# naba89/EDM-TTS

Measured on NVIDIA B200. Metric: s2a_decoded_codec_frames_per_s, higher is better.
Workload: dtype bf16

## Files before the change

edm_tts_b200/csrc/abi.cu:

```cuda
#include <atomic>
#include <cmath>
#include <cstdarg>
#include <cstdio>
#include <cstdlib>
#include <cstring>
#include <string>
#include <algorithm>
#include <utility>
#include <vector>

#include "../../include/edm_s2a.h"
#include "attention.cuh"
#include "elementwise.cuh"
#include "conv_stream.cuh"
#include "dac_conv.cuh"
#include "gemm.cuh"
#include "kmeans.cuh"
#include "rvq_tc.cuh"

using namespace edm;

namespace {

thread_local char g_err[512] = "";
// ... 135 lines not shown
  cfg.stream = st;
  cudaLaunchAttribute attr[1];
  attr[0].id = cudaLaunchAttributeProgrammaticStreamSerialization;
  attr[0].val.programmaticStreamSerializationAllowed = 1;
  cfg.attrs = attr;
  cfg.numAttrs = pdl_enabled() ? 1 : 0;
  cudaLaunchKernelEx(&cfg, kernel, std::forward<Args>(args)...);
}

typedef CUresult (*PFN_tmapEncodeTiled)(CUtensorMap*, CUtensorMapDataType, cuuint32_t, void*, const cuuint64_t*, const cuuint64_t*,
                                        const cuuint32_t*, const cuuint32_t*, CUtensorMapInterleave, CUtensorMapSwizzle,
                                        CUtensorMapL2promotion, CUtensorMapFloatOOBfill);
PFN_tmapEncodeTiled get_encode() {
  static PFN_tmapEncodeTiled fn = nullptr;
  if (fn == nullptr) {
    void* p = nullptr;
    cudaDriverEntryPointQueryResult q;
    if (cudaGetDriverEntryPoint("cuTensorMapEncodeTiled", &p, cudaEnableDefault, &q) == cudaSuccess && q == cudaDriverEntryPointSuccess)
      fn = reinterpret_cast<PFN_tmapEncodeTiled>(p);
  }
  return fn;
}

int make_tmap_2d(CUtensorMap* m, const void* ptr, uint64_t rows, uint64_t cols, uint64_t ld, uint32_t box_rows) {
  PFN_tmapEncodeTiled enc = get_encode();
  if (enc == nullptr) return fail(EDM_ERR_CUDA, "cuTensorMapEncodeTiled entry point not available");
  if ((reinterpret_cast<uintptr_t>(ptr) & 15) != 0 || (ld * 2) % 16 != 0) return fail(EDM_ERR_INVALID, "TMA operand must be 16-byte aligned (ptr %p, ld %llu)", ptr, (unsigned long long)ld);
  cuuint64_t dims[2] = {cols, rows};
  cuuint64_t strides[1] = {ld * 2};
  cuuint32_t box[2] = {64, box_rows};
  cuuint32_t estr[2] = {1, 1};
  CUresult r = enc(m, CU_TENSOR_MAP_DATA_TYPE_BFLOAT16, 2, const_cast<void*>(ptr), dims, strides, box, estr, CU_TENSOR_MAP_INTERLEAVE_NONE,
                   CU_TENSOR_MAP_SWIZZLE_128B, CU_TENSOR_MAP_L2_PROMOTION_L2_256B, CU_TENSOR_MAP_FLOAT_OOB_FILL_NONE);
  if (r != CUDA_SUCCESS) return fail(EDM_ERR_CUDA, "cuTensorMapEncodeTiled(2d rows=%llu cols=%llu ld=%llu) failed: %d", (unsigned long long)rows, (unsigned long long)cols, (unsigned long long)ld, (int)r);
  return 0;
}
int make_tmap_f32_2d(CUtensorMap* m, const void* ptr, uint64_t rows, uint64_t cols, uint64_t ld, uint32_t box_rows,
                     CUtensorMapSwizzle swizzle = CU_TENSOR_MAP_SWIZZLE_128B) {
  PFN_tmapEncodeTiled enc = get_encode();
  if (enc == nullptr) return fail(EDM_ERR_CUDA, "cuTensorMapEncodeTiled entry point not available");
  if ((reinterpret_cast<uintptr_t>(ptr) & 15) != 0 || (ld * 4) % 16 != 0) return fail(EDM_ERR_INVALID, "TMA operand must be 16-byte aligned (ptr %p, ld %llu)", ptr, (unsigned long long)ld);
  cuuint64_t dims[2] = {cols, rows};
  cuuint64_t strides[1] = {ld * 4};
  cuuint32_t box[2] = {32, box_rows};
  cuuint32_t estr[2] = {1, 1};
  CUresult r = enc(m, CU_TENSOR_MAP_DATA_TYPE_FLOAT32, 2, const_cast<void*>(ptr), dims, strides, box, estr, CU_TENSOR_MAP_INTERLEAVE_NONE,
                   swizzle, CU_TENSOR_MAP_L2_PROMOTION_L2_256B, CU_TENSOR_MAP_FLOAT_OOB_FILL_NONE);
  if (r != CUDA_SUCCESS) return fail(EDM_ERR_CUDA, "cuTensorMapEncodeTiled(f32 rows=%llu cols=%llu ld=%llu) failed: %d", (unsigned long long)rows, (unsigned long long)cols, (unsigned long long)ld, (int)r);
  return 0;
}

int next_direction() {
  static const bool enabled = env_switch("EDM_FLIP", true);
  thread_local int dir = 0;
  if (!enabled) return 0;
  dir ^= 1;
  return dir;
}

struct WMap {
  CUtensorMap big, small;
};
int make_wmap(WMap* m, const void* ptr, uint64_t rows, uint64_t cols, uint64_t ld) {
  if (rows % kGemmBN == 0) {
    if (int rc = make_tmap_2d(&m->big, ptr, rows, cols, ld, kGemmBN / 2)) return rc;
  } else {
    memset(&m->big, 0, sizeof(m->big));
  }
  return make_tmap_2d(&m->small, ptr, rows, cols, ld, kSmBN);
}
bool gemm_small_m() { static const bool v = env_switch("EDM_GEMM_SMALL", true); return v; }
bool gemm_resid_tma() { static const bool v = env_switch("EDM_RESID_TMA", true); return v; }
int resid_tma_max_k() { static const int v = env_int("EDM_RESID_TMA_MAXK", 2048); return v; }
bool gemm_out_tma() { static const bool v = env_switch("EDM_OUT_TMA", true); return v; }

template <int EPI>
int launch_gemm_t(const CUtensorMap& ma, const WMap& wm, const GemmParams& p_in, cudaStream_t st) {
  const CUtensorMap& mb = wm.big;
  GemmParams p = p_in;
  p.reverse = next_direction();
  static DeviceOnce attr_once;
  if (attr_once.needed()) {
    EDM_CUDA(cudaFuncSetAttribute(gemm_bf16_tn_pair_kernel<EPI>, cudaFuncAttributeMaxDynamicSharedMemorySize, kPairSmemBytes));
    EDM_CUDA(cudaFuncSetAttribute(gemm_bf16_tn_small_kernel<EPI>, cudaFuncAttributeMaxDynamicSharedMemorySize, kSmSmemBytes));
    if (EPI == EPI_RESID_F32)
      EDM_CUDA(cudaFuncSetAttribute(gemm_bf16_tn_pair_kernel<EPI_RESID_TMA>, cudaFuncAttributeMaxDynamicSharedMemorySize, kPairSmemBytes));
    if (EPI == EPI_SWISH_BF16)
      EDM_CUDA(cudaFuncSetAttribute(gemm_bf16_tn_pair_kernel<EPI_SWISH_TMA>, cudaFuncAttributeMaxDynamicSharedMemorySize, kPairSmemBytes));
    if (EPI == EPI_QKV_ROPE)
      EDM_CUDA(cudaFuncSetAttribute(gemm_bf16_tn_pair_kernel<EPI_ROPE_TMA>, cudaFuncAttributeMaxDynamicSharedMemorySize, kPairSmemBytes));
    if (EPI == EPI_F32)
      EDM_CUDA(cudaFuncSetAttribute(gemm_bf16_tn_pair_kernel<EPI_F32_TMA>, cudaFuncAttributeMaxDynamicSharedMemorySize, kPairSmemBytes));
    attr_once.done();
  }
  ProfScope prof(PK_GEMM, 2.0 * p.M * p.N * p.K, st);
  const int sms = num_sms();
  {
    const int pair_tiles = ((p.M + 2 * kGemmBM - 1) / (2 * kGemmBM)) * ((p.N + kGemmBN - 1) / kGemmBN);
    if (p.N % kGemmBN != 0 || (gemm_small_m() && pair_tiles * 4 <= sms)) {
      p.reverse = 0;
      const int tiles = ((p.M + kGemmBM - 1) / kGemmBM) * (p.N / kSmBN);
      launch_pdl(gemm_bf16_tn_small_kernel<EPI>, dim3(tiles < sms ? tiles : sms), dim3(kSmThreads), kSmSmemBytes, st, ma, wm.small, p);
      EDM_LAUNCH_CHECK("gemm_bf16_tn_small");
      return 0;
    }
  }
  const int tiles = ((p.M + 2 * kGemmBM - 1) / (2 * kGemmBM)) * (p.N / kGemmBN);
  const int pairs = tiles < sms / 2 ? tiles : sms / 2;
  if (EPI == EPI_RESID_F32 && gemm_resid_tma() && p.K <= resid_tma_max_k() && (reinterpret_cast<uintptr_t>(p.out) & 15) == 0 && (p.ldo * 4) % 16 == 0) {
    CUtensorMap mc;
    if (int rc = make_tmap_f32_2d(&mc, p.out, p.M, p.N, p.ldo, 32, CU_TENSOR_MAP_SWIZZLE_128B)) return rc;
    launch_pdl(gemm_bf16_tn_pair_kernel<EPI_RESID_TMA>, dim3(2 * pairs), dim3(kGemmThreads), kPairSmemBytes, st, ma, mb, mc, p);
  } else if (EPI == EPI_F32 && gemm_out_tma() && (reinterpret_cast<uintptr_t>(p.out) & 15) == 0 && (p.ldo * 4) % 16 == 0) {
    CUtensorMap mc;
    if (int rc = make_tmap_f32_2d(&mc, p.out, p.M, p.N, p.ldo, 32, CU_TENSOR_MAP_SWIZZLE_128B)) return rc;
    launch_pdl(gemm_bf16_tn_pair_kernel<EPI_F32_TMA>, dim3(2 * pairs), dim3(kGemmThreads), kPairSmemBytes, st, ma, mb, mc, p);
  } else if ((EPI == EPI_SWISH_BF16 || EPI == EPI_QKV_ROPE) && gemm_out_tma() && (reinterpret_cast<uintptr_t>(p.out) & 15) == 0 && (p.ldo * 2) % 16 == 0) {
    CUtensorMap mc;
    if (int rc = make_tmap_2d(&mc, p.out, p.M, p.N, p.ldo, 32)) return rc;
    if (EPI == EPI_SWISH_BF16)
      launch_pdl(gemm_bf16_tn_pair_kernel<EPI_SWISH_TMA>, dim3(2 * pairs), dim3(kGemmThreads), kPairSmemBytes, st, ma, mb, mc, p);
    else
      launch_pdl(gemm_bf16_tn_pair_kernel<EPI_ROPE_TMA>, dim3(2 * pairs), dim3(kGemmThreads), kPairSmemBytes, st, ma, mb, mc, p);
  } else {
    launch_pdl(gemm_bf16_tn_pair_kernel<EPI>, dim3(2 * pairs), dim3(kGemmThreads), kPairSmemBytes, st, ma, mb, ma, p);
  }
  EDM_LAUNCH_CHECK("gemm_bf16_tn_pair");
  return 0;
}
int launch_gemm(int epi, const CUtensorMap& ma, const WMap& mb, const GemmParams& p, cudaStream_t st) {
  if (p.M <= 0 || p.N <= 0 || p.N % kSmBN != 0 || p.N > kGemmMaxN || p.K % kGemmBK != 0 || p.K <= 0) return fail(EDM_ERR_INVALID, "gemm shape M=%d N=%d K=%d unsupported (N %% 64, N <= 8192, K %% 64)", p.M, p.N, p.K);
  switch (epi) {
    case EPI_BF16: return launch_gemm_t<EPI_BF16>(ma, mb, p, st);
    case EPI_SWISH_BF16: return launch_gemm_t<EPI_SWISH_BF16>(ma, mb, p, st);
    case EPI_QKV_ROPE: return launch_gemm_t<EPI_QKV_ROPE>(ma, mb, p, st);
    case EPI_RESID_F32: return launch_gemm_t<EPI_RESID_F32>(ma, mb, p, st);
    case EPI_F32: return launch_gemm_t<EPI_F32>(ma, mb, p, st);
    case EPI_GLU_BF16: return launch_gemm_t<EPI_GLU_BF16>(ma, mb, p, st);
    case EPI_ARGMAX: return launch_gemm_t<EPI_ARGMAX>(ma, mb, p, st);
  }
  return fail(EDM_ERR_INVALID, "unknown epilogue %d", epi);
}

#ifdef EDM_ATTN_TRACE
unsigned long long* g_attn_trace = nullptr;
#endif
int launch_attention(const CUtensorMap& mqkv, const SeqLayout& lay, const int* pairs, int n_pairs, double flops, int H, void* out, uint32_t lbo,
                     uint32_t sbo, uint32_t kstep, cudaStream_t st, float scale = 0.125f) {
// ... 179 lines not shown
  for (auto& e : g_prof) {
    g_event_pool.push_back(e.a);
    g_event_pool.push_back(e.b);
  }
  g_prof.clear();
  g_prof_on = on != 0;
}
extern "C" int edm_prof_collect(double* ms, double* work, int* count) {
  for (int k = 0; k < PK_COUNT; ++k) {
    ms[k] = 0.0;
    work[k] = 0.0;
    count[k] = 0;
  }
  for (auto& e : g_prof) {
    EDM_CUDA(cudaEventSynchronize(e.b));
    float t = 0.f;
    EDM_CUDA(cudaEventElapsedTime(&t, e.a, e.b));
    ms[e.kind] += t;
    work[e.kind] += e.work;
    count[e.kind] += 1;
  }
  return 0;
}

#ifdef EDM_KTRACE
extern "C" int edm_ktrace_dump(unsigned long long* host, int max_slots) {
  unsigned n = 0;
  cudaDeviceSynchronize();
  cudaMemcpyFromSymbol(&n, g_ktrace_n, sizeof(n));
  const int m = static_cast<int>(n) < max_slots ? static_cast<int>(n) : max_slots;
  if (host != nullptr && m > 0) cudaMemcpyFromSymbol(host, g_ktrace, sizeof(unsigned long long) * 8 * (m < 4096 ? m : 4096));
  const unsigned zero = 0;
  cudaMemcpyToSymbol(g_ktrace_n, &zero, sizeof(zero));
  return static_cast<int>(n);
}
#endif

extern "C" int edm_gemm_bf16(const void* a, long long lda, const void* b, long long ldb, int M, int N, int K, int epilogue,
                             const float* bias, void* out, long long ldo, float scale, const float* rope_cos,
                             const float* rope_sin, int seq_len, int rope_cols, void* stream) {
  if (int rc = check_arch()) return rc;
  CUtensorMap ma;
  WMap mb;
  if (int rc = make_tmap_2d(&ma, a, M, K, lda, kGemmBM)) return rc;
  if (int rc = make_wmap(&mb, b, N, K, ldb)) return rc;
  GemmParams p;
// ... 1722 lines not shown
```

edm_tts_b200/csrc/gemm.cuh:

```cuda
#pragma once
#include "ptx.cuh"
#include "seq_layout.cuh"

namespace edm {

enum EpiKind : int {
  EPI_BF16 = 0,
  EPI_SWISH_BF16 = 1,
  EPI_QKV_ROPE = 2,
  EPI_RESID_F32 = 3,
  EPI_F32 = 4,
  EPI_GLU_BF16 = 5,
  EPI_ARGMAX = 10,
  EPI_F32_TMA = 9,
  EPI_ROPE_TMA = 8,
  EPI_SWISH_TMA = 7,
  EPI_RESID_TMA = 6,
};

struct GemmParams {
  int M, N, K;
  int a_k_offset;
  int b_row_offset;
  const float* bias;
// ... 70 lines not shown
  for (int i = 0; i < 32; ++i)
    if (b[i] > best) {
      best = b[i];
      idx = 32 + i;
    }
  float2* o = reinterpret_cast<float2*>(p.out) + static_cast<long long>(row) * p.ldo + (col >> 6);
  *o = make_float2(best, __int_as_float(col + idx));
}

__device__ __forceinline__ void gemm_store_glu(const GemmParams& p, int row, int col_out, const float (&a)[32], const float (&g)[32]) {
  uint32_t w[16];
#pragma unroll
  for (int i = 0; i < 16; ++i) {
    const uint32_t a2 = pack_bf16x2(a[2 * i], a[2 * i + 1]);
    const uint32_t g2 = pack_bf16x2(g[2 * i], g[2 * i + 1]);
    const uint32_t s2 = pack_bf16x2(sigmoid_tanh(bf16lo(g2)), sigmoid_tanh(bf16hi(g2)));
    w[i] = bf16x2_mul(a2, s2);
  }
  uint4* o = reinterpret_cast<uint4*>(static_cast<__nv_bfloat16*>(p.out) + static_cast<long long>(row) * p.ldo + col_out);
#pragma unroll
  for (int i = 0; i < 4; ++i) o[i] = make_uint4(w[4 * i], w[4 * i + 1], w[4 * i + 2], w[4 * i + 3]);
}

__device__ __forceinline__ void gemm_epilogue_rope64(const GemmParams& p, int row, int col, const uint32_t (&lo)[32],
                                                     const uint32_t (&hi)[32], uint32_t tab_row = 0, int swz = 0, uint32_t stg_row = 0) {
  uint4* o = reinterpret_cast<uint4*>(static_cast<__nv_bfloat16*>(p.out) + static_cast<long long>(row) * p.ldo + col);
  auto put = [&](int c, uint4 v) {
    if (stg_row != 0)
      sts128(stg_row + ((c ^ swz) << 4), make_float4(__uint_as_float(v.x), __uint_as_float(v.y), __uint_as_float(v.z), __uint_as_float(v.w)));
    else
      o[c] = v;
  };
  uint32_t l2[16], h2[16];
#pragma unroll
  for (int i = 0; i < 16; ++i) {
    l2[i] = pack_bf16x2(__uint_as_float(lo[2 * i]), __uint_as_float(lo[2 * i + 1]));
    h2[i] = pack_bf16x2(__uint_as_float(hi[2 * i]), __uint_as_float(hi[2 * i + 1]));
  }
  if (col < p.rope_cols) {
    const int pos = rope_pos(p, row);
    const float4* c4 = reinterpret_cast<const float4*>(p.rope_cos + static_cast<long long>(pos) * 32);
    const float4* s4 = reinterpret_cast<const float4*>(p.rope_sin + static_cast<long long>(pos) * 32);
#pragma unroll
    for (int g = 0; g < 4; ++g) {
      float4 cs[2], sn[2];
      if (tab_row != 0) {
        cs[0] = lds128(tab_row + 16 * ((2 * g) ^ swz));
        cs[1] = lds128(tab_row + 16 * ((2 * g + 1) ^ swz));
        sn[0] = lds128(tab_row + 16 * (8 + ((2 * g) ^ swz)));
        sn[1] = lds128(tab_row + 16 * (8 + ((2 * g + 1) ^ swz)));
      } else {
        cs[0] = __ldg(c4 + 2 * g);
        cs[1] = __ldg(c4 + 2 * g + 1);
        sn[0] = __ldg(s4 + 2 * g);
        sn[1] = __ldg(s4 + 2 * g + 1);
      }
      uint32_t ol[4], oh[4];
#pragma unroll
      for (int q = 0; q < 4; ++q) {
        const int i = 4 * g + q;
        const float4 c = cs[q >> 1], s = sn[q >> 1];
        const float c0 = (q & 1) ? c.z : c.x, c1 = (q & 1) ? c.w : c.y;
        const float s0 = (q & 1) ? s.z : s.x, s1 = (q & 1) ? s.w : s.y;
        const float x1a = bf16lo(l2[i]), x1b = bf16hi(l2[i]), x2a = bf16lo(h2[i]), x2b = bf16hi(h2[i]);
        ol[q] = pack_bf16x2(__fadd_rn(__fmul_rn(x1a, c0), __fmul_rn(-x2a, s0)), __fadd_rn(__fmul_rn(x1b, c1), __fmul_rn(-x2b, s1)));
        oh[q] = pack_bf16x2(__fadd_rn(__fmul_rn(x2a, c0), __fmul_rn(x1a, s0)), __fadd_rn(__fmul_rn(x2b, c1), __fmul_rn(x1b, s1)));
      }
      put(g, make_uint4(ol[0], ol[1], ol[2], ol[3]));
      put(4 + g, make_uint4(oh[0], oh[1], oh[2], oh[3]));
    }
  } else {
#pragma unroll
    for (int g = 0; g < 4; ++g) {
      put(g, make_uint4(l2[4 * g], l2[4 * g + 1], l2[4 * g + 2], l2[4 * g + 3]));
      put(4 + g, make_uint4(h2[4 * g], h2[4 * g + 1], h2[4 * g + 2], h2[4 * g + 3]));
    }
  }
}

constexpr int kSmBN = 64;
constexpr int kSmStages = 8;
constexpr int kSmThreads = 64 + 32 * 4;
constexpr uint32_t kSmBBytes = kSmBN * kGemmBK * 2;
constexpr uint32_t kSmStageBytes = kGemmABytes + kSmBBytes;
constexpr uint32_t kSmSmemBytes = kSmStages * kSmStageBytes + 1024 + 256;

template <int EPI>
__global__ void __launch_bounds__(kSmThreads, 1)
gemm_bf16_tn_small_kernel(const __grid_constant__ CUtensorMap tma_a, const __grid_constant__ CUtensorMap tma_b, const GemmParams p) {
  extern __shared__ uint8_t smem_raw[];
  uint8_t* smem = reinterpret_cast<uint8_t*>((reinterpret_cast<uintptr_t>(smem_raw) + 1023) & ~static_cast<uintptr_t>(1023));
  uint64_t* full_bar = reinterpret_cast<uint64_t*>(smem + kSmStages * kSmStageBytes);
  uint64_t* empty_bar = full_bar + kSmStages;
  uint64_t* tmem_full_bar = empty_bar + kSmStages;
  uint64_t* tmem_empty_bar = tmem_full_bar + 2;
  uint32_t* tmem_base_slot = reinterpret_cast<uint32_t*>(tmem_empty_bar + 2);

  const int warp = threadIdx.x >> 5;
  const int lane = threadIdx.x & 31;
  const int num_m = (p.M + kGemmBM - 1) / kGemmBM;
// ... 99 lines not shown
      }
      if constexpr (EPI != EPI_QKV_ROPE) {
        const float4* bg = reinterpret_cast<const float4*>(p.bias != nullptr ? p.bias + col0 : nullptr);
#pragma unroll
        for (int i = 0; i < 16; ++i) bias_v[i] = bg != nullptr ? __ldg(bg + i) : make_float4(0.f, 0.f, 0.f, 0.f);
      }
      mbar_wait(&tmem_full_bar[acc], acc_phase);
      tc_fence_after();
      uint32_t r0[32], r1[32];
      tmem_ld_32x32(taddr, r0);
      tmem_ld_32x32(taddr + 32, r1);
      tmem_ld_wait_dep(r0);
      tmem_ld_wait_dep(r1);
      tc_fence_before();
      __syncwarp();
#ifdef EDM_KTRACE
      if (warp == 2 && lane == 0) KTRACE_PUT(5, ktrace_now());
#endif
      if (lane == 0) mbar_arrive(&tmem_empty_bar[acc]);
      acc ^= 1;
      if (acc == 0) acc_phase ^= 1;
      if (row >= p.M) continue;
      if constexpr (EPI == EPI_QKV_ROPE) {
        gemm_epilogue_rope64(p, row, col0, r0, r1);
      } else {
        auto bias4 = [&](int i) { return bias_v[i]; };
        float v[32];
#pragma unroll
        for (int i = 0; i < 8; ++i) {
          const float4 b = bias4(i);
          v[4 * i + 0] = __uint_as_float(r0[4 * i + 0]) + b.x;
          v[4 * i + 1] = __uint_as_float(r0[4 * i + 1]) + b.y;
          v[4 * i + 2] = __uint_as_float(r0[4 * i + 2]) + b.z;
          v[4 * i + 3] = __uint_as_float(r0[4 * i + 3]) + b.w;
        }
        if constexpr (EPI == EPI_GLU_BF16 || EPI == EPI_ARGMAX) {
          float g[32];
#pragma unroll
          for (int i = 0; i < 8; ++i) {
            const float4 b = bias4(8 + i);
            g[4 * i + 0] = __uint_as_float(r1[4 * i + 0]) + b.x;
            g[4 * i + 1] = __uint_as_float(r1[4 * i + 1]) + b.y;
            g[4 * i + 2] = __uint_as_float(r1[4 * i + 2]) + b.z;
            g[4 * i + 3] = __uint_as_float(r1[4 * i + 3]) + b.w;
          }
          if constexpr (EPI == EPI_GLU_BF16)
            gemm_store_glu(p, row, col0 >> 1, v, g);
// ... 6 lines not shown
#pragma unroll
          for (int i = 0; i < 8; ++i) {
            const float4 b = bias4(8 + i);
            v[4 * i + 0] = __uint_as_float(r1[4 * i + 0]) + b.x;
            v[4 * i + 1] = __uint_as_float(r1[4 * i + 1]) + b.y;
            v[4 * i + 2] = __uint_as_float(r1[4 * i + 2]) + b.z;
            v[4 * i + 3] = __uint_as_float(r1[4 * i + 3]) + b.w;
          }
          gemm_store_32<EPI>(q, row, col0 + 32, v);
        }
      }
    }
  }

  tc_fence_before();
  __syncthreads();
#ifdef EDM_KTRACE
  if (threadIdx.x == 64) KTRACE_END(100 + EPI);
#endif
  if (warp == 1) tmem_dealloc<128>(tmem_base);
}

constexpr uint32_t kPairStageBytes = 2 * kGemmABytes;
constexpr uint32_t kPairStagingBytes = 32 * 32 * 4;
constexpr uint32_t kPairRopeTabBytes = 128 * 16 * 16;
constexpr uint32_t kPairBarOffset = 7 * kPairStageBytes;
constexpr uint32_t kPairSmemBytes = kPairBarOffset + 256 + 1024;
__host__ __device__ constexpr int pair_stages(bool tma_out, bool rope) { return rope ? (tma_out ? 4 : 6) : (tma_out ? 5 : 7); }
constexpr int kPairMaxStages = 7;

template <int EPI>
__global__ void __cluster_dims__(2, 1, 1) __launch_bounds__(kGemmThreads, 1)
gemm_bf16_tn_pair_kernel(const __grid_constant__ CUtensorMap tma_a, const __grid_constant__ CUtensorMap tma_b,
                         const __grid_constant__ CUtensorMap tma_c, const GemmParams p) {
  constexpr bool kTmaOut = EPI == EPI_RESID_TMA || EPI == EPI_SWISH_TMA || EPI == EPI_ROPE_TMA || EPI == EPI_F32_TMA;
  constexpr bool kRope = EPI == EPI_QKV_ROPE || EPI == EPI_ROPE_TMA;
  constexpr int kSt = pair_stages(kTmaOut, kRope);
  constexpr uint32_t kStagingOffset = kSt * kPairStageBytes;
  constexpr uint32_t kRopeTabOffset = kStagingOffset + (kTmaOut ? kGemmEpiWarps * kPairStagingBytes : 0);
  static_assert(kRopeTabOffset + (kRope ? kPairRopeTabBytes : 0) <= kPairBarOffset, "smem budget");
  extern __shared__ uint8_t smem_raw[];
  uint8_t* smem = reinterpret_cast<uint8_t*>((reinterpret_cast<uintptr_t>(smem_raw) + 1023) & ~static_cast<uintptr_t>(1023));
  float* s_rope = reinterpret_cast<float*>(smem + kRopeTabOffset);
  uint64_t* full_bar = reinterpret_cast<uint64_t*>(smem + kPairBarOffset);
  uint64_t* empty_bar = full_bar + kPairMaxStages;
  uint64_t* tmem_full_bar = empty_bar + kPairMaxStages;
  uint64_t* tmem_empty_bar = tmem_full_bar + 2;
  uint32_t* tmem_base_slot = reinterpret_cast<uint32_t*>(tmem_empty_bar + 2);

  const int warp = threadIdx.x >> 5;
  const int lane = threadIdx.x & 31;
  const uint32_t rank = cluster_ctarank();
  const int pair = blockIdx.x >> 1, num_pairs = gridDim.x >> 1;

  const int num_m = (p.M + 2 * kGemmBM - 1) / (2 * kGemmBM);
  const int num_n = p.N / kGemmBN;
  const int num_tiles = num_m * num_n;
  const int num_kb = p.K / kGemmBK;

  if (warp == 0 && lane == 0) {
    tma_prefetch_desc(&tma_a);
    tma_prefetch_desc(&tma_b);
    for (int s = 0; s < kSt; ++s) {
      mbar_init(&full_bar[s], 1);
      mbar_init(&empty_bar[s], 1);
    }
    for (int b = 0; b < 2; ++b) {
      mbar_init(&tmem_full_bar[b], 1);
      mbar_init(&tmem_empty_bar[b], 2 * kGemmEpiWarps);
    }
    fence_mbar_init();
  }
  if (warp == 1) tmem_alloc_pair<512>(tmem_base_slot);
  tc_fence_before();
  cluster_sync_all();
  tc_fence_after();
  const uint32_t tmem_base = *tmem_base_slot;
  pdl_sync();

  if (warp == 0) {
    if (lane == 0) {
      int stage = 0;
      uint32_t phase = 0;
      for (int t = pair; t < num_tiles; t += num_pairs) {
        const int tt = p.reverse ? num_tiles - 1 - t : t;
        const int m_blk = tt / num_n, n_blk = tt % num_n;
        for (int kb = 0; kb < num_kb; ++kb) {
          mbar_wait(&empty_bar[stage], phase ^ 1);
          uint8_t* sa = smem + stage * kPairStageBytes;
          uint8_t* sb = sa + kGemmABytes;
          if (rank == 0) mbar_arrive_expect_tx(&full_bar[stage], 2 * kPairStageBytes);
          tma_load_2d_pair(&tma_a, &full_bar[stage], sa, p.a_k_offset + kb * kGemmBK, m_blk * 2 * kGemmBM + rank * kGemmBM);
          tma_load_2d_pair(&tma_b, &full_bar[stage], sb, kb * kGemmBK, p.b_row_offset + n_blk * kGemmBN + rank * (kGemmBN / 2));
          if (++stage == kSt) {
            stage = 0;
            phase ^= 1;
          }
        }
      }
    }
  } else if (warp == 1) {
    if (rank == 0) {
      constexpr uint32_t idesc = umma_idesc_bf16(2 * kGemmBM, kGemmBN, 0, 0);
      int stage = 0;
      uint32_t phase = 0;
      int acc = 0;
      uint32_t acc_phase = 0;
      for (int t = pair; t < num_tiles; t += num_pairs) {
        mbar_wait(&tmem_empty_bar[acc], acc_phase ^ 1);
        tc_fence_after();
        const uint32_t d_tmem = tmem_base + acc * kGemmBN;
        for (int kb = 0; kb < num_kb; ++kb) {
          mbar_wait(&full_bar[stage], phase);
          tc_fence_after();
          const uint32_t sa = smem_u32(smem + stage * kPairStageBytes);
          const uint64_t adesc = umma_desc_sw128(sa, 16, 1024);
          const uint64_t bdesc = umma_desc_sw128(sa + kGemmABytes, 16, 1024);
#pragma unroll
          for (int k = 0; k < kGemmBK / 16; ++k) umma_ss_pair_warp(d_tmem, adesc + 2 * k, bdesc + 2 * k, idesc, (kb | k) != 0 ? 1u : 0u);
          umma_commit_pair_warp(&empty_bar[stage]);
          if (++stage == kSt) {
            stage = 0;
            phase ^= 1;
          }
        }
        umma_commit_pair_warp(&tmem_full_bar[acc]);
        acc ^= 1;
        if (acc == 0) acc_phase ^= 1;
      }
    }
  } else {
    const int quad = warp & 3;
    const int sub = (warp - 2) >> 2;
    int acc = 0;
    uint32_t acc_phase = 0;
    for (int t = pair; t < num_tiles; t += num_pairs) {
      const int tt = p.reverse ? num_tiles - 1 - t : t;
      const int m_blk = tt / num_n, n_blk = tt % num_n;
      const int row = m_blk * 2 * kGemmBM + static_cast<int>(rank) * kGemmBM + quad * 32 + lane;
      const int col0 = n_blk * kGemmBN + sub * 64;
      const uint32_t taddr = tmem_base + (static_cast<uint32_t>(quad * 32) << 16) + acc * kGemmBN + sub * 64;
      const float4* bias_g = reinterpret_cast<const float4*>(p.bias != nullptr ? p.bias + col0 : nullptr);
      auto bias4 = [&](int k) { return bias_g != nullptr ? __ldg(bias_g + k) : make_float4(0.f, 0.f, 0.f, 0.f); };
      bool rope_tile = false;
      if constexpr (kRope) {
        rope_tile = n_blk * kGemmBN < p.rope_cols;
        if (rope_tile) {
          float4* tab = reinterpret_cast<float4*>(s_rope);
          const int et = threadIdx.x - 64;
          asm volatile("bar.sync 1, 512;" ::: "memory");
#pragma unroll
          for (int i = et; i < 128 * 16; i += 32 * kGemmEpiWarps) {
            const int r = i >> 4, c = i & 15;
            const int grow = m_blk * 2 * kGemmBM + static_cast<int>(rank) * kGemmBM + r;
            const int pos = rope_pos(p, grow < p.M ? grow : 0);
            const float* src = (c < 8 ? p.rope_cos : p.rope_sin) + static_cast<long long>(pos) * 32 + (c & 7) * 4;
            tab[r * 16 + (c ^ (r & 7))] = __ldg(reinterpret_cast<const float4*>(src));
          }
          asm volatile("bar.sync 1, 512;" ::: "memory");
        }
      }
      mbar_wait(&tmem_full_bar[acc], acc_phase);
      tc_fence_after();
      uint32_t r0[32], r1[32];
      tmem_ld_32x32(taddr, r0);
      tmem_ld_32x32(taddr + 32, r1);
      tmem_ld_wait_dep(r0);
      tmem_ld_wait_dep(r1);
      tc_fence_before();
      __syncwarp();
      if (lane == 0) mbar_arrive_cluster(&tmem_empty_bar[acc], 0);
      acc ^= 1;
      if (acc == 0) acc_phase ^= 1;
      if constexpr (EPI == EPI_ROPE_TMA) {
        uint8_t* stg = smem + kStagingOffset + (warp - 2) * kPairStagingBytes;
        const int tr = quad * 32 + lane;
        if (lane == 0) bulk_wait_group_read0();
        __syncwarp();
        gemm_epilogue_rope64(p, row, col0, r0, r1, rope_tile ? smem_u32(s_rope) + tr * 256 : 0u, tr & 7, smem_u32(stg) + lane * 128);
        fence_proxy_async_smem();
        __syncwarp();
        if (lane == 0) {
          tma_store_2d(&tma_c, stg, col0, m_blk * 2 * kGemmBM + static_cast<int>(rank) * kGemmBM + quad * 32);
          bulk_commit_group();
        }
        continue;
      }
      if constexpr (EPI == EPI_SWISH_TMA) {
        uint8_t* stg = smem + kStagingOffset + (warp - 2) * kPairStagingBytes;
        const uint32_t stg_row = smem_u32(stg) + lane * 128;
        const int sw = lane & 7;
        const int row0 = m_blk * 2 * kGemmBM + static_cast<int>(rank) * kGemmBM + quad * 32;
        uint32_t w[32];
#pragma unroll
        for (int h = 0; h < 2; ++h) {
          const uint32_t* r = h == 0 ? r0 : r1;
#pragma unroll
          for (int i = 0; i < 8; ++i) {
            const float4 b = bias4(8 * h + i);
            const uint32_t h01 = pack_bf16x2(__uint_as_float(r[4 * i + 0]) + b.x, __uint_as_float(r[4 * i + 1]) + b.y);
            const uint32_t h23 = pack_bf16x2(__uint_as_float(r[4 * i + 2]) + b.z, __uint_as_float(r[4 * i + 3]) + b.w);
            w[16 * h + 2 * i] = bf16x2_mul(h01, pack_bf16x2(sigmoid_tanh(bf16lo(h01)), sigmoid_tanh(bf16hi(h01))));
            w[16 * h + 2 * i + 1] = bf16x2_mul(h23, pack_bf16x2(sigmoid_tanh(bf16lo(h23)), sigmoid_tanh(bf16hi(h23))));
          }
        }
        if (lane == 0) bulk_wait_group_read0();
        __syncwarp();
#pragma unroll
        for (int c = 0; c < 8; ++c)
          sts128(stg_row + ((c ^ sw) << 4), make_float4(__uint_as_float(w[4 * c]), __uint_as_float(w[4 * c + 1]), __uint_as_float(w[4 * c + 2]),
                                                       __uint_as_float(w[4 * c + 3])));
        fence_proxy_async_smem();
        __syncwarp();
        if (lane == 0) {
          tma_store_2d(&tma_c, stg, col0, row0);
          bulk_commit_group();
        }
        continue;
      }
      if constexpr (EPI == EPI_RESID_TMA || EPI == EPI_F32_TMA) {
        uint8_t* stg = smem + kStagingOffset + (warp - 2) * kPairStagingBytes;
        const uint32_t stg_row = smem_u32(stg) + lane * 128;
        const int sw = lane & 7;
        const int row0 = m_blk * 2 * kGemmBM + static_cast<int>(rank) * kGemmBM + quad * 32;
#pragma unroll
        for (int h = 0; h < 2; ++h) {
          if (lane == 0) bulk_wait_group_read0();
          __syncwarp();
#pragma unroll
          for (int i = 0; i < 8; ++i) {
            const float4 b = bias4(8 * h + i);
            const uint32_t* r = h == 0 ? r0 : r1;
            if constexpr (EPI == EPI_RESID_TMA)
              sts128(stg_row + ((i ^ sw) << 4),
                     make_float4(p.scale * bf16_round(__uint_as_float(r[4 * i + 0]) + b.x), p.scale * bf16_round(__uint_as_float(r[4 * i + 1]) + b.y),
                                 p.scale * bf16_round(__uint_as_float(r[4 * i + 2]) + b.z), p.scale * bf16_round(__uint_as_float(r[4 * i + 3]) + b.w)));
            else
              sts128(stg_row + ((i ^ sw) << 4), make_float4(__uint_as_float(r[4 * i + 0]) + b.x, __uint_as_float(r[4 * i + 1]) + b.y,
                                                            __uint_as_float(r[4 * i + 2]) + b.z, __uint_as_float(r[4 * i + 3]) + b.w));
          }
          fence_proxy_async_smem();
          __syncwarp();
          if (lane == 0) {
            if constexpr (EPI == EPI_RESID_TMA)
              tma_reduce_add_2d(&tma_c, stg, col0 + 32 * h, row0);
            else
              tma_store_2d(&tma_c, stg, col0 + 32 * h, row0);
            bulk_commit_group();
          }
        }
        continue;
      }
      if (row >= p.M) continue;
      if constexpr (EPI == EPI_QKV_ROPE) {
        const int tr = quad * 32 + lane;
        gemm_epilogue_rope64(p, row, col0, r0, r1, rope_tile ? smem_u32(s_rope) + tr * 256 : 0u, tr & 7);
      } else {
        float v[32];
#pragma unroll
        for (int i = 0; i < 8; ++i) {
          const float4 b = bias4(i);
          v[4 * i + 0] = __uint_as_float(r0[4 * i + 0]) + b.x;
          v[4 * i + 1] = __uint_as_float(r0[4 * i + 1]) + b.y;
          v[4 * i + 2] = __uint_as_float(r0[4 * i + 2]) + b.z;
          v[4 * i + 3] = __uint_as_float(r0[4 * i + 3]) + b.w;
        }
        if constexpr (EPI == EPI_GLU_BF16 || EPI == EPI_ARGMAX) {
          float g[32];
#pragma unroll
          for (int i = 0; i < 8; ++i) {
            const float4 b = bias4(8 + i);
            g[4 * i + 0] = __uint_as_float(r1[4 * i + 0]) + b.x;
            g[4 * i + 1] = __uint_as_float(r1[4 * i + 1]) + b.y;
            g[4 * i + 2] = __uint_as_float(r1[4 * i + 2]) + b.z;
            g[4 * i + 3] = __uint_as_float(r1[4 * i + 3]) + b.w;
          }
          if constexpr (EPI == EPI_GLU_BF16)
            gemm_store_glu(p, row, col0 >> 1, v, g);
          else
            gemm_store_argmax(p, row, col0, v, g);
        } else {
          gemm_store_32<EPI>(p, row, col0, v);
#pragma unroll
          for (int i = 0; i < 8; ++i) {
            const float4 b = bias4(8 + i);
            v[4 * i + 0] = __uint_as_float(r1[4 * i + 0]) + b.x;
            v[4 * i + 1] = __uint_as_float(r1[4 * i + 1]) + b.y;
            v[4 * i + 2] = __uint_as_float(r1[4 * i + 2]) + b.z;
            v[4 * i + 3] = __uint_as_float(r1[4 * i + 3]) + b.w;
          }
          gemm_store_32<EPI>(p, row, col0 + 32, v);
        }
      }
    }
  }

  if constexpr (kTmaOut) {
    if (warp >= 2 && lane == 0) bulk_wait_group0();
  }
  tc_fence_before();
  cluster_sync_all();
  if (warp == 1) tmem_dealloc_pair<512>(tmem_base);
}

}
```

Measured before the change: 292,200.

## Shrink bf16 epilogue staging to deepen pair GEMM pipeline and drop rope smem table

Bf16 TMA-output epilogues (swish and rope) now stage 32x32 bf16 halves with 64B swizzle instead of a full 64-column tile. Pipeline stage count is derived from leftover shared memory, so these kernels get more mainloop stages. The shared-memory rope cos/sin table and its named barriers are replaced by per-thread L1 prefetch and direct global loads. The changes add an extra TMA store per tile and more global traffic for the rope tables. Optional trace counters and a stage-override debug path are added behind compile flags.

```diff
diff --git a/edm_tts_b200/csrc/abi.cu b/edm_tts_b200/csrc/abi.cu
--- a/edm_tts_b200/csrc/abi.cu
+++ b/edm_tts_b200/csrc/abi.cu
@@ -181,16 +181,16 @@
   return fn;
 }
 
-int make_tmap_2d(CUtensorMap* m, const void* ptr, uint64_t rows, uint64_t cols, uint64_t ld, uint32_t box_rows) {
+int make_tmap_2d(CUtensorMap* m, const void* ptr, uint64_t rows, uint64_t cols, uint64_t ld, uint32_t box_rows, uint32_t box_cols = 64) {
   PFN_tmapEncodeTiled enc = get_encode();
   if (enc == nullptr) return fail(EDM_ERR_CUDA, "cuTensorMapEncodeTiled entry point not available");
   if ((reinterpret_cast<uintptr_t>(ptr) & 15) != 0 || (ld * 2) % 16 != 0) return fail(EDM_ERR_INVALID, "TMA operand must be 16-byte aligned (ptr %p, ld %llu)", ptr, (unsigned long long)ld);
   cuuint64_t dims[2] = {cols, rows};
   cuuint64_t strides[1] = {ld * 2};
-  cuuint32_t box[2] = {64, box_rows};
+  cuuint32_t box[2] = {box_cols, box_rows};
   cuuint32_t estr[2] = {1, 1};
   CUresult r = enc(m, CU_TENSOR_MAP_DATA_TYPE_BFLOAT16, 2, const_cast<void*>(ptr), dims, strides, box, estr, CU_TENSOR_MAP_INTERLEAVE_NONE,
-                   CU_TENSOR_MAP_SWIZZLE_128B, CU_TENSOR_MAP_L2_PROMOTION_L2_256B, CU_TENSOR_MAP_FLOAT_OOB_FILL_NONE);
+                   box_cols == 64 ? CU_TENSOR_MAP_SWIZZLE_128B : CU_TENSOR_MAP_SWIZZLE_64B, CU_TENSOR_MAP_L2_PROMOTION_L2_256B, CU_TENSOR_MAP_FLOAT_OOB_FILL_NONE);
   if (r != CUDA_SUCCESS) return fail(EDM_ERR_CUDA, "cuTensorMapEncodeTiled(2d rows=%llu cols=%llu ld=%llu) failed: %d", (unsigned long long)rows, (unsigned long long)cols, (unsigned long long)ld, (int)r);
   return 0;
 }
@@ -232,6 +232,24 @@
 bool gemm_resid_tma() { static const bool v = env_switch("EDM_RESID_TMA", true); return v; }
 int resid_tma_max_k() { static const int v = env_int("EDM_RESID_TMA_MAXK", 2048); return v; }
 bool gemm_out_tma() { static const bool v = env_switch("EDM_OUT_TMA", true); return v; }
+
+template <int EPI>
+void launch_pair(int pairs, cudaStream_t st, const CUtensorMap& ma, const CUtensorMap& mb, const CUtensorMap& mc, const GemmParams& p) {
+#ifdef EDM_BRINGUP
+  static const int stages = env_int("EDM_PAIR_STAGES", 0);
+  if (stages >= 4 && stages < pair_stages(EPI)) {
+    auto go = [&](auto kernel) {
+      cudaFuncSetAttribute(kernel, cudaFuncAttributeMaxDynamicSharedMemorySize, kPairSmemBytes);
+      launch_pdl(kernel, dim3(2 * pairs), dim3(kGemmThreads), kPairSmemBytes, st, ma, mb, mc, p);
+    };
+    if (stages == 4) go(gemm_bf16_tn_pair_kernel<EPI, 4>);
+    if constexpr (pair_stages(EPI) > 5) if (stages == 5) go(gemm_bf16_tn_pair_kernel<EPI, 5>);
+    if constexpr (pair_stages(EPI) > 6) if (stages == 6) go(gemm_bf16_tn_pair_kernel<EPI, 6>);
+    return;
+  }
+#endif
+  launch_pdl(gemm_bf16_tn_pair_kernel<EPI>, dim3(2 * pairs), dim3(kGemmThreads), kPairSmemBytes, st, ma, mb, mc, p);
+}
 
 template <int EPI>
 int launch_gemm_t(const CUtensorMap& ma, const WMap& wm, const GemmParams& p_in, cudaStream_t st) {
@@ -269,20 +287,20 @@
   if (EPI == EPI_RESID_F32 && gemm_resid_tma() && p.K <= resid_tma_max_k() && (reinterpret_cast<uintptr_t>(p.out) & 15) == 0 && (p.ldo * 4) % 16 == 0) {
     CUtensorMap mc;
     if (int rc = make_tmap_f32_2d(&mc, p.out, p.M, p.N, p.ldo, 32, CU_TENSOR_MAP_SWIZZLE_128B)) return rc;
-    launch_pdl(gemm_bf16_tn_pair_kernel<EPI_RESID_TMA>, dim3(2 * pairs), dim3(kGemmThreads), kPairSmemBytes, st, ma, mb, mc, p);
+    launch_pair<EPI_RESID_TMA>(pairs, st, ma, mb, mc, p);
   } else if (EPI == EPI_F32 && gemm_out_tma() && (reinterpret_cast<uintptr_t>(p.out) & 15) == 0 && (p.ldo * 4) % 16 == 0) {
     CUtensorMap mc;
     if (int rc = make_tmap_f32_2d(&mc, p.out, p.M, p.N, p.ldo, 32, CU_TENSOR_MAP_SWIZZLE_128B)) return rc;
-    launch_pdl(gemm_bf16_tn_pair_kernel<EPI_F32_TMA>, dim3(2 * pairs), dim3(kGemmThreads), kPairSmemBytes, st, ma, mb, mc, p);
+    launch_pair<EPI_F32_TMA>(pairs, st, ma, mb, mc, p);
   } else if ((EPI == EPI_SWISH_BF16 || EPI == EPI_QKV_ROPE) && gemm_out_tma() && (reinterpret_cast<uintptr_t>(p.out) & 15) == 0 && (p.ldo * 2) % 16 == 0) {
     CUtensorMap mc;
-    if (int rc = make_tmap_2d(&mc, p.out, p.M, p.N, p.ldo, 32)) return rc;
+    if (int rc = make_tmap_2d(&mc, p.out, p.M, p.N, p.ldo, 32, 32)) return rc;
     if (EPI == EPI_SWISH_BF16)
-      launch_pdl(gemm_bf16_tn_pair_kernel<EPI_SWISH_TMA>, dim3(2 * pairs), dim3(kGemmThreads), kPairSmemBytes, st, ma, mb, mc, p);
+      launch_pair<EPI_SWISH_TMA>(pairs, st, ma, mb, mc, p);
     else
-      launch_pdl(gemm_bf16_tn_pair_kernel<EPI_ROPE_TMA>, dim3(2 * pairs), dim3(kGemmThreads), kPairSmemBytes, st, ma, mb, mc, p);
+      launch_pair<EPI_ROPE_TMA>(pairs, st, ma, mb, mc, p);
   } else {
-    launch_pdl(gemm_bf16_tn_pair_kernel<EPI>, dim3(2 * pairs), dim3(kGemmThreads), kPairSmemBytes, st, ma, mb, ma, p);
+    launch_pair<EPI>(pairs, st, ma, mb, ma, p);
   }
   EDM_LAUNCH_CHECK("gemm_bf16_tn_pair");
   return 0;
@@ -508,6 +526,24 @@
   }
   return 0;
 }
+
+#ifdef EDM_BRINGUP
+extern "C" int edm_pair_stages_dbg(int epi) {
+  const int own = pair_stages(epi), over = env_int("EDM_PAIR_STAGES", 0);
+  return over >= 4 && over < own ? over : own;
+}
+#endif
+
+#ifdef EDM_PAIR_TRACE
+extern "C" int edm_pair_trace_dump(unsigned long long* host, int max_ctas) {
+  static unsigned long long zero[8 * 1024];
+  const int n = max_ctas < 1024 ? max_ctas : 1024;
+  cudaDeviceSynchronize();
+  if (host != nullptr && n > 0) cudaMemcpyFromSymbol(host, g_pair_trace, sizeof(unsigned long long) * 8 * n);
+  cudaMemcpyToSymbol(g_pair_trace, zero, sizeof(zero));
+  return cudaDeviceSynchronize() == cudaSuccess ? 0 : 1;
+}
+#endif
 
 #ifdef EDM_KTRACE
 extern "C" int edm_ktrace_dump(unsigned long long* host, int max_slots) {
diff --git a/edm_tts_b200/csrc/gemm.cuh b/edm_tts_b200/csrc/gemm.cuh
--- a/edm_tts_b200/csrc/gemm.cuh
+++ b/edm_tts_b200/csrc/gemm.cuh
@@ -116,15 +116,8 @@
   for (int i = 0; i < 4; ++i) o[i] = make_uint4(w[4 * i], w[4 * i + 1], w[4 * i + 2], w[4 * i + 3]);
 }
 
-__device__ __forceinline__ void gemm_epilogue_rope64(const GemmParams& p, int row, int col, const uint32_t (&lo)[32],
-                                                     const uint32_t (&hi)[32], uint32_t tab_row = 0, int swz = 0, uint32_t stg_row = 0) {
-  uint4* o = reinterpret_cast<uint4*>(static_cast<__nv_bfloat16*>(p.out) + static_cast<long long>(row) * p.ldo + col);
-  auto put = [&](int c, uint4 v) {
-    if (stg_row != 0)
-      sts128(stg_row + ((c ^ swz) << 4), make_float4(__uint_as_float(v.x), __uint_as_float(v.y), __uint_as_float(v.z), __uint_as_float(v.w)));
-    else
-      o[c] = v;
-  };
+__device__ __forceinline__ void gemm_rope64(const GemmParams& p, int row, int col, const uint32_t (&lo)[32], const uint32_t (&hi)[32],
+                                            uint32_t (&o)[32]) {
   uint32_t l2[16], h2[16];
 #pragma unroll
   for (int i = 0; i < 16; ++i) {
@@ -132,24 +125,13 @@
     h2[i] = pack_bf16x2(__uint_as_float(hi[2 * i]), __uint_as_float(hi[2 * i + 1]));
   }
   if (col < p.rope_cols) {
-    const int pos = rope_pos(p, row);
+    const int pos = rope_pos(p, row < p.M ? row : 0);
     const float4* c4 = reinterpret_cast<const float4*>(p.rope_cos + static_cast<long long>(pos) * 32);
     const float4* s4 = reinterpret_cast<const float4*>(p.rope_sin + static_cast<long long>(pos) * 32);
 #pragma unroll
     for (int g = 0; g < 4; ++g) {
-      float4 cs[2], sn[2];
-      if (tab_row != 0) {
-        cs[0] = lds128(tab_row + 16 * ((2 * g) ^ swz));
-        cs[1] = lds128(tab_row + 16 * ((2 * g + 1) ^ swz));
-        sn[0] = lds128(tab_row + 16 * (8 + ((2 * g) ^ swz)));
-        sn[1] = lds128(tab_row + 16 * (8 + ((2 * g + 1) ^ swz)));
-      } else {
-        cs[0] = __ldg(c4 + 2 * g);
-        cs[1] = __ldg(c4 + 2 * g + 1);
-        sn[0] = __ldg(s4 + 2 * g);
-        sn[1] = __ldg(s4 + 2 * g + 1);
-      }
-      uint32_t ol[4], oh[4];
+      const float4 cs[2] = {__ldg(c4 + 2 * g), __ldg(c4 + 2 * g + 1)};
+      const float4 sn[2] = {__ldg(s4 + 2 * g), __ldg(s4 + 2 * g + 1)};
 #pragma unroll
       for (int q = 0; q < 4; ++q) {
         const int i = 4 * g + q;
@@ -157,19 +139,23 @@
         const float c0 = (q & 1) ? c.z : c.x, c1 = (q & 1) ? c.w : c.y;
         const float s0 = (q & 1) ? s.z : s.x, s1 = (q & 1) ? s.w : s.y;
         const float x1a = bf16lo(l2[i]), x1b = bf16hi(l2[i]), x2a = bf16lo(h2[i]), x2b = bf16hi(h2[i]);
-        ol[q] = pack_bf16x2(__fadd_rn(__fmul_rn(x1a, c0), __fmul_rn(-x2a, s0)), __fadd_rn(__fmul_rn(x1b, c1), __fmul_rn(-x2b, s1)));
-        oh[q] = pack_bf16x2(__fadd_rn(__fmul_rn(x2a, c0), __fmul_rn(x1a, s0)), __fadd_rn(__fmul_rn(x2b, c1), __fmul_rn(x1b, s1)));
-      }
-      put(g, make_uint4(ol[0], ol[1], ol[2], ol[3]));
-      put(4 + g, make_uint4(oh[0], oh[1], oh[2], oh[3]));
+        o[i] = pack_bf16x2(__fadd_rn(__fmul_rn(x1a, c0), __fmul_rn(-x2a, s0)), __fadd_rn(__fmul_rn(x1b, c1), __fmul_rn(-x2b, s1)));
+        o[16 + i] = pack_bf16x2(__fadd_rn(__fmul_rn(x2a, c0), __fmul_rn(x1a, s0)), __fadd_rn(__fmul_rn(x2b, c1), __fmul_rn(x1b, s1)));
+      }
     }
   } else {
 #pragma unroll
-    for (int g = 0; g < 4; ++g) {
-      put(g, make_uint4(l2[4 * g], l2[4 * g + 1], l2[4 * g + 2], l2[4 * g + 3]));
-      put(4 + g, make_uint4(h2[4 * g], h2[4 * g + 1], h2[4 * g + 2], h2[4 * g + 3]));
-    }
-  }
+    for (int i = 0; i < 16; ++i) {
+      o[i] = l2[i];
+      o[16 + i] = h2[i];
+    }
+  }
+}
+
+__device__ __forceinline__ void gemm_store_bf16x64(const GemmParams& p, int row, int col, const uint32_t (&w)[32]) {
+  uint4* o = reinterpret_cast<uint4*>(static_cast<__nv_bfloat16*>(p.out) + static_cast<long long>(row) * p.ldo + col);
+#pragma unroll
+  for (int i = 0; i < 8; ++i) o[i] = make_uint4(w[4 * i], w[4 * i + 1], w[4 * i + 2], w[4 * i + 3]);
 }
 
 constexpr int kSmBN = 64;
@@ -315,7 +301,9 @@
       if (acc == 0) acc_phase ^= 1;
       if (row >= p.M) continue;
       if constexpr (EPI == EPI_QKV_ROPE) {
-        gemm_epilogue_rope64(p, row, col0, r0, r1);
+        uint32_t w[32];
+        gemm_rope64(p, row, col0, r0, r1, w);
+        gemm_store_bf16x64(p, row, col0, w);
       } else {
         auto bias4 = [&](int i) { return bias_v[i]; };
         float v[32];
@@ -368,26 +356,33 @@
 }
 
 constexpr uint32_t kPairStageBytes = 2 * kGemmABytes;
-constexpr uint32_t kPairStagingBytes = 32 * 32 * 4;
-constexpr uint32_t kPairRopeTabBytes = 128 * 16 * 16;
 constexpr uint32_t kPairBarOffset = 7 * kPairStageBytes;
 constexpr uint32_t kPairSmemBytes = kPairBarOffset + 256 + 1024;
-__host__ __device__ constexpr int pair_stages(bool tma_out, bool rope) { return rope ? (tma_out ? 4 : 6) : (tma_out ? 5 : 7); }
 constexpr int kPairMaxStages = 7;
-
-template <int EPI>
+__host__ __device__ constexpr uint32_t pair_staging_bytes(int epi) {
+  return (epi == EPI_RESID_TMA || epi == EPI_F32_TMA) ? 32 * 32 * 4 : (epi == EPI_SWISH_TMA || epi == EPI_ROPE_TMA) ? 32 * 32 * 2 : 0;
+}
+__host__ __device__ constexpr int pair_stages(int epi) {
+  return static_cast<int>((kPairBarOffset - kGemmEpiWarps * pair_staging_bytes(epi)) / kPairStageBytes);
+}
+
+#ifdef EDM_PAIR_TRACE
+__device__ unsigned long long g_pair_trace[8 * 1024];
+#define PAIR_TRACE(...) __VA_ARGS__
+#else
+#define PAIR_TRACE(...)
+#endif
+
+template <int EPI, int kSt = pair_stages(EPI)>
 __global__ void __cluster_dims__(2, 1, 1) __launch_bounds__(kGemmThreads, 1)
 gemm_bf16_tn_pair_kernel(const __grid_constant__ CUtensorMap tma_a, const __grid_constant__ CUtensorMap tma_b,
                          const __grid_constant__ CUtensorMap tma_c, const GemmParams p) {
-  constexpr bool kTmaOut = EPI == EPI_RESID_TMA || EPI == EPI_SWISH_TMA || EPI == EPI_ROPE_TMA || EPI == EPI_F32_TMA;
-  constexpr bool kRope = EPI == EPI_QKV_ROPE || EPI == EPI_ROPE_TMA;
-  constexpr int kSt = pair_stages(kTmaOut, kRope);
+  constexpr bool kTmaOut = pair_staging_bytes(EPI) != 0;
+  constexpr uint32_t kStg = pair_staging_bytes(EPI);
   constexpr uint32_t kStagingOffset = kSt * kPairStageBytes;
-  constexpr uint32_t kRopeTabOffset = kStagingOffset + (kTmaOut ? kGemmEpiWarps * kPairStagingBytes : 0);
-  static_assert(kRopeTabOffset + (kRope ? kPairRopeTabBytes : 0) <= kPairBarOffset, "smem budget");
+  static_assert(kSt <= kPairMaxStages && kStagingOffset + kGemmEpiWarps * kStg <= kPairBarOffset, "smem budget");
   extern __shared__ uint8_t smem_raw[];
   uint8_t* smem = reinterpret_cast<uint8_t*>((reinterpret_cast<uintptr_t>(smem_raw) + 1023) & ~static_cast<uintptr_t>(1023));
-  float* s_rope = reinterpret_cast<float*>(smem + kRopeTabOffset);
   uint64_t* full_bar = reinterpret_cast<uint64_t*>(smem + kPairBarOffset);
   uint64_t* empty_bar = full_bar + kPairMaxStages;
   uint64_t* tmem_full_bar = empty_bar + kPairMaxStages;
@@ -423,6 +418,7 @@
   tc_fence_after();
   const uint32_t tmem_base = *tmem_base_slot;
   pdl_sync();
+  PAIR_TRACE(unsigned long long tr_ns0; asm volatile("mov.u64 %0, %%globaltimer;" : "=l"(tr_ns0)); const long long tr_c0 = clock64();)
 
   if (warp == 0) {
     if (lane == 0) {
@@ -452,12 +448,17 @@
       uint32_t phase = 0;
       int acc = 0;
       uint32_t acc_phase = 0;
+      PAIR_TRACE(long long tr_full = 0, tr_empty = 0, tr_tiles = 0, tr_t; const long long tr_start = clock64();)
       for (int t = pair; t < num_tiles; t += num_pairs) {
+        PAIR_TRACE(tr_t = clock64();)
         mbar_wait(&tmem_empty_bar[acc], acc_phase ^ 1);
+        PAIR_TRACE(tr_empty += clock64() - tr_t; ++tr_tiles;)
         tc_fence_after();
         const uint32_t d_tmem = tmem_base + acc * kGemmBN;
         for (int kb = 0; kb < num_kb; ++kb) {
+          PAIR_TRACE(tr_t = clock64();)
           mbar_wait(&full_bar[stage], phase);
+          PAIR_TRACE(tr_full += clock64() - tr_t;)
           tc_fence_after();
           const uint32_t sa = smem_u32(smem + stage * kPairStageBytes);
           const uint64_t adesc = umma_desc_sw128(sa, 16, 1024);
@@ -474,13 +475,22 @@
         acc ^= 1;
         if (acc == 0) acc_phase ^= 1;
       }
+      PAIR_TRACE(if (lane == 0) {
+        unsigned long long* tr = g_pair_trace + 8 * blockIdx.x;
+        atomicAdd(tr + 0, tr_full);
+        atomicAdd(tr + 1, tr_empty);
+        atomicAdd(tr + 2, tr_tiles);
+        atomicAdd(tr + 3, clock64() - tr_start);
+      })
     }
   } else {
     const int quad = warp & 3;
     const int sub = (warp - 2) >> 2;
     int acc = 0;
     uint32_t acc_phase = 0;
+    PAIR_TRACE(long long tr_wait = 0, tr_work = 0, tr_rel = 0;)
     for (int t = pair; t < num_tiles; t += num_pairs) {
+      PAIR_TRACE(const long long tr_top = clock64(); if (tr_rel != 0) tr_work += tr_top - tr_rel;)
       const int tt = p.reverse ? num_tiles - 1 - t : t;
       const int m_blk = tt / num_n, n_blk = tt % num_n;
       const int row = m_blk * 2 * kGemmBM + static_cast<int>(rank) * kGemmBM + quad * 32 + lane;
@@ -488,22 +498,10 @@
       const uint32_t taddr = tmem_base + (static_cast<uint32_t>(quad * 32) << 16) + acc * kGemmBN + sub * 64;
       const float4* bias_g = reinterpret_cast<const float4*>(p.bias != nullptr ? p.bias + col0 : nullptr);
       auto bias4 = [&](int k) { return bias_g != nullptr ? __ldg(bias_g + k) : make_float4(0.f, 0.f, 0.f, 0.f); };
-      bool rope_tile = false;
-      if constexpr (kRope) {
-        rope_tile = n_blk * kGemmBN < p.rope_cols;
-        if (rope_tile) {
-          float4* tab = reinterpret_cast<float4*>(s_rope);
-          const int et = threadIdx.x - 64;
-          asm volatile("bar.sync 1, 512;" ::: "memory");
-#pragma unroll
-          for (int i = et; i < 128 * 16; i += 32 * kGemmEpiWarps) {
-            const int r = i >> 4, c = i & 15;
-            const int grow = m_blk * 2 * kGemmBM + static_cast<int>(rank) * kGemmBM + r;
-            const int pos = rope_pos(p, grow < p.M ? grow : 0);
-            const float* src = (c < 8 ? p.rope_cos : p.rope_sin) + static_cast<long long>(pos) * 32 + (c & 7) * 4;
-            tab[r * 16 + (c ^ (r & 7))] = __ldg(reinterpret_cast<const float4*>(src));
-          }
-          asm volatile("bar.sync 1, 512;" ::: "memory");
+      if constexpr (EPI == EPI_QKV_ROPE || EPI == EPI_ROPE_TMA) {
+        if (col0 < p.rope_cols && row < p.M) {
+          prefetch_l1(p.rope_cos + static_cast<long long>(rope_pos(p, row)) * 32);
+          prefetch_l1(p.rope_sin + static_cast<long long>(rope_pos(p, row)) * 32);
         }
       }
       mbar_wait(&tmem_full_bar[acc], acc_phase);
@@ -516,56 +514,50 @@
       tc_fence_before();
       __syncwarp();
       if (lane == 0) mbar_arrive_cluster(&tmem_empty_bar[acc], 0);
+      PAIR_TRACE(tr_rel = clock64(); tr_wait += tr_rel - tr_top;)
       acc ^= 1;
       if (acc == 0) acc_phase ^= 1;
-      if constexpr (EPI == EPI_ROPE_TMA) {
-        uint8_t* stg = smem + kStagingOffset + (warp - 2) * kPairStagingBytes;
-        const int tr = quad * 32 + lane;
-        if (lane == 0) bulk_wait_group_read0();
-        __syncwarp();
-        gemm_epilogue_rope64(p, row, col0, r0, r1, rope_tile ? smem_u32(s_rope) + tr * 256 : 0u, tr & 7, smem_u32(stg) + lane * 128);
-        fence_proxy_async_smem();
-        __syncwarp();
-        if (lane == 0) {
-          tma_store_2d(&tma_c, stg, col0, m_blk * 2 * kGemmBM + static_cast<int>(rank) * kGemmBM + quad * 32);
-          bulk_commit_group();
+      if constexpr (EPI == EPI_ROPE_TMA || EPI == EPI_SWISH_TMA) {
+        uint32_t w[32];
+        if constexpr (EPI == EPI_ROPE_TMA) {
+          gemm_rope64(p, row, col0, r0, r1, w);
+        } else {
+#pragma unroll
+          for (int h = 0; h < 2; ++h) {
+            const uint32_t* r = h == 0 ? r0 : r1;
+#pragma unroll
+            for (int i = 0; i < 8; ++i) {
+              const float4 b = bias4(8 * h + i);
+              const uint32_t h01 = pack_bf16x2(__uint_as_float(r[4 * i + 0]) + b.x, __uint_as_float(r[4 * i + 1]) + b.y);
+              const uint32_t h23 = pack_bf16x2(__uint_as_float(r[4 * i + 2]) + b.z, __uint_as_float(r[4 * i + 3]) + b.w);
+              w[16 * h + 2 * i] = bf16x2_mul(h01, pack_bf16x2(sigmoid_tanh(bf16lo(h01)), sigmoid_tanh(bf16hi(h01))));
+              w[16 * h + 2 * i + 1] = bf16x2_mul(h23, pack_bf16x2(sigmoid_tanh(bf16lo(h23)), sigmoid_tanh(bf16hi(h23))));
+            }
+          }
+        }
+        uint8_t* stg = smem + kStagingOffset + (warp - 2) * kStg;
+        const uint32_t stg_row = smem_u32(stg) + lane * 64;
+        const int sw = (lane >> 1) & 3;
+        const int row0 = m_blk * 2 * kGemmBM + static_cast<int>(rank) * kGemmBM + quad * 32;
+#pragma unroll
+        for (int h = 0; h < 2; ++h) {
+          if (lane == 0) bulk_wait_group_read0();
+          __syncwarp();
+#pragma unroll
+          for (int c = 0; c < 4; ++c)
+            sts128(stg_row + ((c ^ sw) << 4), make_float4(__uint_as_float(w[16 * h + 4 * c]), __uint_as_float(w[16 * h + 4 * c + 1]),
+                                                         __uint_as_float(w[16 * h + 4 * c + 2]), __uint_as_float(w[16 * h + 4 * c + 3])));
+          fence_proxy_async_smem();
+          __syncwarp();
+          if (lane == 0) {
+            tma_store_2d(&tma_c, stg, col0 + 32 * h, row0);
+            bulk_commit_group();
+          }
         }
         continue;
       }
-      if constexpr (EPI == EPI_SWISH_TMA) {
-        uint8_t* stg = smem + kStagingOffset + (warp - 2) * kPairStagingBytes;
-        const uint32_t stg_row = smem_u32(stg) + lane * 128;
-        const int sw = lane & 7;
-        const int row0 = m_blk * 2 * kGemmBM + static_cast<int>(rank) * kGemmBM + quad * 32;
-        uint32_t w[32];
-#pragma unroll
-        for (int h = 0; h < 2; ++h) {
-          const uint32_t* r = h == 0 ? r0 : r1;
-#pragma unroll
-          for (int i = 0; i < 8; ++i) {
-            const float4 b = bias4(8 * h + i);
-            const uint32_t h01 = pack_bf16x2(__uint_as_float(r[4 * i + 0]) + b.x, __uint_as_float(r[4 * i + 1]) + b.y);
-            const uint32_t h23 = pack_bf16x2(__uint_as_float(r[4 * i + 2]) + b.z, __uint_as_float(r[4 * i + 3]) + b.w);
-            w[16 * h + 2 * i] = bf16x2_mul(h01, pack_bf16x2(sigmoid_tanh(bf16lo(h01)), sigmoid_tanh(bf16hi(h01))));
-            w[16 * h + 2 * i + 1] = bf16x2_mul(h23, pack_bf16x2(sigmoid_tanh(bf16lo(h23)), sigmoid_tanh(bf16hi(h23))));
-          }
-        }
-        if (lane == 0) bulk_wait_group_read0();
-        __syncwarp();
-#pragma unroll
-        for (int c = 0; c < 8; ++c)
-          sts128(stg_row + ((c ^ sw) << 4), make_float4(__uint_as_float(w[4 * c]), __uint_as_float(w[4 * c + 1]), __uint_as_float(w[4 * c + 2]),
-                                                       __uint_as_float(w[4 * c + 3])));
-        fence_proxy_async_smem();
-        __syncwarp();
-        if (lane == 0) {
-          tma_store_2d(&tma_c, stg, col0, row0);
-          bulk_commit_group();
-        }
-        continue;
-      }
       if constexpr (EPI == EPI_RESID_TMA || EPI == EPI_F32_TMA) {
-        uint8_t* stg = smem + kStagingOffset + (warp - 2) * kPairStagingBytes;
+        uint8_t* stg = smem + kStagingOffset + (warp - 2) * kStg;
         const uint32_t stg_row = smem_u32(stg) + lane * 128;
         const int sw = lane & 7;
         const int row0 = m_blk * 2 * kGemmBM + static_cast<int>(rank) * kGemmBM + quad * 32;
@@ -599,8 +591,9 @@
       }
       if (row >= p.M) continue;
       if constexpr (EPI == EPI_QKV_ROPE) {
-        const int tr = quad * 32 + lane;
-        gemm_epilogue_rope64(p, row, col0, r0, r1, rope_tile ? smem_u32(s_rope) + tr * 256 : 0u, tr & 7);
+        uint32_t w[32];
+        gemm_rope64(p, row, col0, r0, r1, w);
+        gemm_store_bf16x64(p, row, col0, w);
       } else {
         float v[32];
 #pragma unroll
@@ -639,6 +632,11 @@
         }
       }
     }
+    PAIR_TRACE(if (warp == 2 && lane == 0) {
+      if (tr_rel != 0) tr_work += clock64() - tr_rel;
+      atomicAdd(g_pair_trace + 8 * blockIdx.x + 4, tr_wait);
+      atomicAdd(g_pair_trace + 8 * blockIdx.x + 5, tr_work);
+    })
   }
 
   if constexpr (kTmaOut) {
@@ -646,6 +644,12 @@
   }
   tc_fence_before();
   cluster_sync_all();
+  PAIR_TRACE(if (threadIdx.x == 0) {
+    unsigned long long ns1;
+    asm volatile("mov.u64 %0, %%globaltimer;" : "=l"(ns1));
+    atomicAdd(g_pair_trace + 8 * blockIdx.x + 6, ns1 - tr_ns0);
+    atomicAdd(g_pair_trace + 8 * blockIdx.x + 7, clock64() - tr_c0);
+  })
   if (warp == 1) tmem_dealloc_pair<512>(tmem_base);
 }
 
```

New measurement: 290,500 (median of 6 runs). About the same (-0.6%).
